# ianic/flate

Measured on AMD Instinct MI355X. Metric: MB/s uncompressed, deflate level 6 compress, higher is better.
Workload: dtype u8; 1 GPU; raw deflate level 6, 1024 MiB synthetic enwik-like text per GPU, 65535-byte independent chunks (16385 chunks), one MI355X per rank (BASELINE.json configs[1]); container=raw, chunk_bytes=65535, bytes_per_gpu=1073741824, gather=none

## Files before the change

### flate_amd/csrc/flate_hip.hip

```cpp
#include <hip/hip_runtime.h>

#include <dlfcn.h>

#include <algorithm>
#include <cstdio>
#include <cstdlib>
#include <cstring>
#include <string>
#include <chrono>
#include <deque>
#include <vector>
#include <thread>
#include <functional>

#include "../../include/flate_hip.h"
#include "kernels_block.h"
#include "kernels_common.h"
#include "kernels_deflater.h"
#include "kernels_inflate.h"
#include "kernels_inflate_par.h"
#include "kernels_inflate_size.h"
#include "kernels_lz.h"
#include "kernels_parse.h"
#include "kernels_walk.h"
// ... 15 lines not shown
    K_LZ_LINKS,
    K_LZ_WALK,
    K_LZ_EMIT,
    K_ST_PARSE,
    K_ST_EMIT,
    K_PLAN,
    K_OFFSETS,
    K_ENCODE,
    K_INFLATE,
    K_INFLATE_PAR,
    K_SPAN_SCAN,
    K_INFLATE_SPAN,
    K_INFLATE_SIZE,
    K_INFLATE_SIZE_SPAN,
    K_GATHER,
    K_INFLATER,
    K_DEFLATER,
    K_COUNT
};
const char* const kKernelNames[K_COUNT] = {"memset_out", "k_byte_hist", "k_checksum", "k_lz_sort", "k_lz_match",
                                           "k_lz_chain", "k_lz_parse", "k_lz_links", "k_lz_walk", "k_lz_emit",
                                           "k_st_parse", "k_st_emit", "k_plan",
                                           "k_offsets",  "k_encode",    "k_inflate",  "k_inflate_par", "k_span_scan", "k_inflate_span",
                                           "k_inflate_size", "k_inflate_size_span",
                                           "k_gather", "k_inflater", "k_deflater"};

struct DevBuf {
    void* p = nullptr;
    size_t cap = 0;
};

}

struct flate_hip_plan {
    std::vector<uint64_t> hin, hout;
    uint32_t n_chunks = 0;
    int container = 0, mode = 0;
    struct Pass {
        uint32_t nc = 0, nb = 0;
        void* chunks = nullptr;
        void* blk_chunk = nullptr;
    };
    std::vector<Pass> passes;
    bool ready = false;
};

struct fl_knobs {
    size_t max_pass_chunks = 32768;
    size_t host_pass_chunks = 1024;
    uint64_t stream_pass_bytes = 4096ull << 20;
    uint64_t span_min_bytes = 0;
    bool span_debug = false;
    int span_twin = -1;
    bool memset_inline = false;
    bool span_two_runs = false;
    bool no_pin_mirror = false;
    bool no_ramp = false;
    uint32_t stream_group = 0;
    int stream_windows = -1;
    bool simple_ck_inline = false;
    bool one_stream = false;
    int rect = -1;
    int64_t inflate_par = -1;
    int64_t inflate_ring = -1;
};

struct flate_hip_ctx {
    int device = 0;
    fl_knobs knobs;
    hipStream_t own_stream = nullptr;
    hipStream_t stream = nullptr;
    bool sync = true;
    uint32_t flags = 0;
    std::string last_error;
    fl_crc_consts crc{};
    DevBuf chunks, blk_chunk, plans, hist, cks, S, NC, rec, desc, marks, tokens, ntok, cflag, links, shard_sz;
    DevBuf wexit;
    DevBuf wchunks, swins;
    void* pin_in = nullptr;
    void* pin_out = nullptr;
    void* pin_len = nullptr;
    void* pin_tab = nullptr;
    size_t pin_tab_cap = 0;
    bool in_mirror = false;
    size_t pin_in_cap = 0, pin_out_cap = 0, pin_len_cap = 0;
    std::function<void(uint32_t, uint32_t)> mirror_in, mirror_out;
    uint32_t n_cu = 0;
    DevBuf sp_points, sp_found, sp_spans, sp_res, sp_cand, sp_candoff, sp_tails, sp_tails_b, sp_chain, sp_chainoff,
        sp_pool, sp_pooltab, sp_poolctl, sp_items, sp_part, sp_footoff, sp_foot, sp_fin, sp_chainpos, sp_rs;
    DevBuf tiles, segs, pieces, fpts, zones, nsorted, jmp, exitmap, entry, segtok, tokbase, bound;
    DevBuf sgroups, sgroup0, gmap, gentry, sblocks;
    DevBuf st_in, st_out, st_inoff, st_outlen, st_status, st_consumed, st_pack, st_packoff, st_slot;
    hipStream_t s_in = nullptr, s_out = nullptr;
    std::vector<hipEvent_t> xfer_events;
    hipStream_t s_ck = nullptr;
    hipEvent_t ck_ev0 = nullptr, ck_ev1 = nullptr;
    hipStream_t s_c2 = nullptr;
    hipEvent_t c2_ev0 = nullptr, c2_ev1 = nullptr;
    hipStream_t s_ms = nullptr;
    hipEvent_t ms_ev0 = nullptr, ms_ev1 = nullptr;
    bool ms_pending = false;
    bool ck_pending = false;
    uint64_t dfl_bytes = 0;
    uint64_t ws_bytes = 0;
    uint64_t dbg_span_taken = 0, dbg_span_done = 0, dbg_par_taken = 0;
    DevBuf dbg_par_handed;
    DevBuf sz_spans, sz_recs;
    uint64_t dbg_size_chain = 0, dbg_size_whole = 0;
    bool ws_fixed = false;
    uint32_t dbg_pass_chunks = 0;
    uint32_t dbg_first_chunk = 0;
    std::vector<uint64_t> dbg_pos_off;
    std::vector<fl_chunk> dbg_chunks;
    std::vector<fl_piece> dbg_pieces;
    bool prof = false;
    struct Pending {
        int kid;
        hipEvent_t a, b;
    };
    std::vector<Pending> pending;
    std::vector<hipEvent_t> free_events;
    double prof_ms[K_COUNT] = {0};
    uint64_t prof_n[K_COUNT] = {0};
};

namespace {

#define HIP_OK(h, expr)                                                                                  \
    do {                                                                                                 \
        hipError_t e_ = (expr);                                                                          \
        if (e_ != hipSuccess) {                                                                          \
            (h)->last_error = std::string(#expr) + ": " + hipGetErrorString(e_);                         \
            return FLATE_HIP_E_LAUNCH;                                                                   \
        }                                                                                                \
    } while (0)

int ensure(flate_hip_ctx* h, DevBuf& b, size_t bytes) {
    if (bytes <= b.cap) return FLATE_HIP_OK;
    if (h->ws_fixed) {
        h->last_error = "workspace of the two-stream passes too small: " + std::to_string(bytes) + " bytes asked, " +
                        std::to_string(b.cap) + " held";
        return FLATE_HIP_E_LAUNCH;
    }
    if (b.p) {
        (void)hipStreamSynchronize(h->stream);
        (void)hipFree(b.p);
        h->ws_bytes -= b.cap;
        b.p = nullptr;
        b.cap = 0;
    }
    size_t want = bytes + bytes / 8 + 256;
    hipError_t e = hipMalloc(&b.p, want);
    if (e != hipSuccess) {
        (void)hipGetLastError();
// ... 45 lines not shown
int launch_checksum_side(flate_hip_ctx* h, uint32_t nb, const uint8_t* d_in, const fl_chunk* dch, const uint32_t* dbc,
                         const fl_sblock* dsb, const fl_params& prm);

void fold_profile(flate_hip_ctx* h) {
    if (h->pending.empty()) return;
    (void)hipStreamSynchronize(h->stream);
    for (auto& p : h->pending) {
        float ms = 0;
        if (hipEventElapsedTime(&ms, p.a, p.b) == hipSuccess) {
            h->prof_ms[p.kid] += ms;
            h->prof_n[p.kid] += 1;
        }
        h->free_events.push_back(p.a);
        h->free_events.push_back(p.b);
    }
    h->pending.clear();
}

void init_crc_consts(fl_crc_consts& cc) {
    cc.xpow8[0] = 0x00800000u;
    for (int j = 1; j < 32; j++) cc.xpow8[j] = fl_crc_mulmod(cc.xpow8[j - 1], cc.xpow8[j - 1]);
    for (int m = 0; m < 64; m++) cc.pow1024[m] = fl_crc_xpow8n(cc.xpow8, 1024ull * m);
    cc.pow65535 = fl_crc_xpow8n(cc.xpow8, 65535);
}

bool level_args(int mode, fl_params& p) {
    switch (mode) {
        case 4: p.good = 4; p.lazy = 4; p.nice = 16; p.chain = 16; return true;
        case 5: p.good = 8; p.lazy = 16; p.nice = 32; p.chain = 32; return true;
        case 6: p.good = 8; p.lazy = 16; p.nice = 128; p.chain = 128; return true;
        case 7: p.good = 8; p.lazy = 32; p.nice = 128; p.chain = 256; return true;
        case 8: p.good = 32; p.lazy = 128; p.nice = 258; p.chain = 1024; return true;
        case 9: p.good = 32; p.lazy = 258; p.nice = 258; p.chain = 4096; return true;
        default: p.good = p.lazy = p.nice = p.chain = 0; return mode == 0 || mode == 1;
    }
}

void read_knobs(fl_knobs& k, uint64_t span_default) {
    k = fl_knobs();
    const char* e;
    if ((e = getenv("FLATE_HIP_MAX_PASS_CHUNKS")) && atoi(e) > 0) k.max_pass_chunks = (size_t)atoi(e);
    if ((e = getenv("FLATE_HIP_HOST_PASS_CHUNKS")) && atoi(e) > 0) k.host_pass_chunks = (size_t)atoi(e);
    if ((e = getenv("FLATE_HIP_MAX_STREAM_PASS_MIB")) && atoll(e) > 0) k.stream_pass_bytes = (uint64_t)atoll(e) << 20;
    e = getenv("FLATE_HIP_INFLATE_SPANS");
    k.span_min_bytes = e ? (uint64_t)atoll(e) : span_default;
    k.span_debug = getenv("FLATE_HIP_SPAN_DEBUG") != nullptr;
    if ((e = getenv("FLATE_HIP_SPAN_TWIN"))) k.span_twin = atoi(e);
    k.no_pin_mirror = getenv("FLATE_HIP_NO_PIN_MIRROR") != nullptr;
    k.no_ramp = getenv("FLATE_HIP_NO_RAMP") != nullptr;
    if ((e = getenv("FLATE_HIP_RECT"))) k.rect = atoi(e) != 0;
    k.one_stream = getenv("FLATE_HIP_ONE_COMPUTE_STREAM") != nullptr;
    k.simple_ck_inline = getenv("FLATE_HIP_SIMPLE_CK_INLINE") != nullptr;
    if ((e = getenv("FLATE_HIP_SPAN_TWO_RUNS"))) k.span_two_runs = atoi(e) != 0;
    if ((e = getenv("FLATE_HIP_MEMSET_INLINE"))) k.memset_inline = atoi(e) != 0;
    if ((e = getenv("FLATE_HIP_STREAM_WINDOWS"))) k.stream_windows = atoi(e) != 0;
    if ((e = getenv("FLATE_HIP_STREAM_GROUP")) && atoi(e) > 0) k.stream_group = (uint32_t)atoi(e);
    if ((e = getenv("FLATE_HIP_INFLATE_PAR"))) k.inflate_par = atoll(e);
    if ((e = getenv("FLATE_HIP_INFLATE_RING"))) k.inflate_ring = atoll(e);
}
size_t pass_chunk_limit(const flate_hip_ctx* h) { return h->knobs.max_pass_chunks; }
size_t host_pass_chunk_limit(const flate_hip_ctx* h) { return h->knobs.host_pass_chunks; }
bool is_pinned_host(const void* p) {
    hipPointerAttribute_t a;
    if (hipPointerGetAttributes(&a, p) != hipSuccess) {
        (void)hipGetLastError();
        return false;
    }
    return a.type == hipMemoryTypeHost;
}
hipError_t create_copy_stream(hipStream_t* s, bool input) {
    int least = 0, greatest = 0;
    if (hipDeviceGetStreamPriorityRange(&least, &greatest) != hipSuccess || least == greatest) {
        (void)hipGetLastError();
        return hipStreamCreateWithFlags(s, hipStreamNonBlocking);
    }
    return hipStreamCreateWithPriority(s, hipStreamNonBlocking, input ? greatest : least);
}

int xfer_event(flate_hip_ctx* h, size_t k, hipEvent_t* ev) {
    while (h->xfer_events.size() <= k) {
        hipEvent_t e;
        if (hipEventCreateWithFlags(&e, hipEventDisableTiming) != hipSuccess) return FLATE_HIP_E_ALLOC;
        h->xfer_events.push_back(e);
    }
    *ev = h->xfer_events[k];
    return FLATE_HIP_OK;
}

uint64_t stream_pass_byte_limit(const flate_hip_ctx* h) { return h->knobs.stream_pass_bytes; }

#ifndef FL_STREAM_FIX_MAX
#define FL_STREAM_FIX_MAX 3u
#endif
int compress_stream_pass(flate_hip_ctx* h, const uint8_t* d_in, const fl_params& prm, uint32_t nc, uint32_t nb,
                         const StreamTables& t, const fl_chunk* hch ) {
    hipStream_t st = h->stream;
    int rc;
    const uint32_t nseg = (uint32_t)t.segs.size(), npc = (uint32_t)t.pieces.size();
    const uint64_t npos = t.npos;
    const size_t tile_limit = pass_chunk_limit(h);
    const size_t tiles_per_launch = std::min(t.tiles.size(), tile_limit);
    if ((rc = ensure(h, h->tiles, sizeof(fl_tile) * t.tiles.size()))) return rc;
    if ((rc = ensure(h, h->segs, sizeof(fl_seg) * (t.segs.size() + 1)))) return rc;
    if ((rc = ensure(h, h->pieces, sizeof(fl_piece) * npc))) return rc;
    if ((rc = ensure(h, h->fpts, sizeof(uint32_t) * (t.fpts.size() + 1)))) return rc;
    if ((rc = ensure(h, h->zones, sizeof(uint32_t) * (t.zones.size() + 1)))) return rc;
    if ((rc = ensure(h, h->nsorted, sizeof(uint32_t) * tiles_per_launch))) return rc;
// ... 336 lines not shown
int launch_checksum_side(flate_hip_ctx* h, uint32_t nb, const uint8_t* d_in, const fl_chunk* dch, const uint32_t* dbc,
                         const fl_sblock* dsb, const fl_params& prm) {
    hipStream_t st = h->stream;
    if (!h->s_ck) {
        hipStream_t s = nullptr;
        hipEvent_t e0 = nullptr, e1 = nullptr;
        if (hipStreamCreateWithFlags(&s, hipStreamNonBlocking) != hipSuccess ||
            hipEventCreateWithFlags(&e0, hipEventDisableTiming) != hipSuccess ||
            hipEventCreateWithFlags(&e1, hipEventDisableTiming) != hipSuccess) {
            if (e0) (void)hipEventDestroy(e0);
            if (e1) (void)hipEventDestroy(e1);
            if (s) (void)hipStreamDestroy(s);
            (void)hipGetLastError();
            return FLATE_HIP_E_ALLOC;
        }
        h->s_ck = s;
        h->ck_ev0 = e0;
        h->ck_ev1 = e1;
    }
    HIP_OK(h, hipEventRecord(h->ck_ev0, st));
    HIP_OK(h, hipStreamWaitEvent(h->s_ck, h->ck_ev0, 0));
    {
        ProfScope ps(h, K_CHECKSUM, h->s_ck);
        hipLaunchKernelGGL(k_checksum, dim3(nb), dim3(64), 0, h->s_ck, d_in, dch, dbc, dsb, prm, h->crc, (uint32_t*)h->cks.p);
    }
    HIP_OK(h, hipEventRecord(h->ck_ev1, h->s_ck));
    h->ck_pending = true;
    return FLATE_HIP_OK;
}

#ifndef FL_ENC_WAVE_MIN_SLOTS_STREAM
#define FL_ENC_WAVE_MIN_SLOTS_STREAM 32768u
#endif
int enqueue_back_end(flate_hip_ctx* h, const fl_params& prm, uint32_t nc, uint32_t nb, uint32_t c0, const fl_chunk* dch,
                     const uint32_t* dbc, const fl_sblock* dsb, const uint8_t* d_in, uint8_t* d_out, uint64_t* d_outlen,
                     int32_t* d_status) {
    hipStream_t st = h->stream;
    const int mode = prm.mode;
    fl_block_plan* dpl = (fl_block_plan*)h->plans.p;
    uint32_t* dhist = (uint32_t*)h->hist.p;
    uint32_t* dcks = (uint32_t*)h->cks.p;
    {
        ProfScope ps(h, K_PLAN);
        if (mode == 0)
            hipLaunchKernelGGL(k_plan_store, dim3((nb + 255) / 256), dim3(256), 0, st, dch, dbc, dsb, nb, dpl);
        else
            hipLaunchKernelGGL(k_plan, dim3((nb + FL_PLAN_WAVES - 1) / FL_PLAN_WAVES), dim3(64 * FL_PLAN_WAVES), 0, st,
                               dch, dbc, dsb, prm, (const uint32_t*)dhist, dpl);
    }
    if (h->ck_pending) {
        HIP_OK(h, hipStreamWaitEvent(st, h->ck_ev1, 0));
        h->ck_pending = false;
    }
    if (h->ms_pending) {
        HIP_OK(h, hipStreamWaitEvent(st, h->ms_ev1, 0));
        h->ms_pending = false;
    }
    {
        ProfScope ps(h, K_OFFSETS);
        hipLaunchKernelGGL(k_offsets, dim3(nc), dim3((uint64_t)nb >= 32ull * nc ? 64 * FL_OFFS_MAX_WAVES : 64), 0, st, dch, prm, h->crc, dpl, (const uint32_t*)dcks,
                           d_out, d_outlen + c0, d_status + c0);
    }
    {
        ProfScope ps(h, K_ENCODE);
        if (mode >= 4 && nb >= (prm.stream ? FL_ENC_WAVE_MIN_SLOTS_STREAM : 8192u))
            hipLaunchKernelGGL(k_encode_wave, dim3((nb + FL_ENC_WAVES - 1) / FL_ENC_WAVES), dim3(64 * FL_ENC_WAVES), 0, st,
                               d_in, dch, dbc, (const fl_block_plan*)dpl, (const uint32_t*)h->tokens.p, (uint32_t*)d_out, nb,
                               (prm.stream || (nb & 1u)) ? 0u : 1u);
        else if (mode >= 4)
            hipLaunchKernelGGL(k_encode<true>, dim3(nb), dim3(64 * FL_ENC_WAVES), 0, st, d_in, dch, dbc,
                               (const fl_block_plan*)dpl, (const uint32_t*)h->tokens.p, (uint32_t*)d_out);
        else
            hipLaunchKernelGGL(k_encode<false>, dim3(nb), dim3(64 * FL_ENC_WAVES), 0, st, d_in, dch, dbc,
                               (const fl_block_plan*)dpl, (const uint32_t*)nullptr, (uint32_t*)d_out);
    }
    HIP_OK(h, hipGetLastError());
    return FLATE_HIP_OK;
}

int enqueue_pass(flate_hip_ctx* h, const fl_params& prm, uint32_t nc, uint32_t nb, uint32_t c0, const fl_chunk* dch,
                 const uint32_t* dbc, const fl_sblock* dsb, const uint8_t* d_in, uint8_t* d_out, uint64_t* d_outlen,
                 int32_t* d_status) {
    hipStream_t st = h->stream;
    const int mode = prm.mode, container = prm.container;
    int rc;
    fl_block_plan* dpl = (fl_block_plan*)h->plans.p;
    uint32_t* dhist = (uint32_t*)h->hist.p;
    if (container != 0 && ((mode >= 4 && prm.chain >= FL_BULK_MIN_CHAIN) || (mode < 4 && h->knobs.simple_ck_inline))) {
        ProfScope ps(h, K_CHECKSUM);
        hipLaunchKernelGGL(k_checksum, dim3(nb), dim3(64), 0, st, d_in, dch, dbc, dsb, prm, h->crc, (uint32_t*)h->cks.p);
    }
    if (container != 0 && mode < 4 && !h->knobs.simple_ck_inline && (rc = launch_checksum_side(h, nb, d_in, dch, dbc, dsb, prm))) return rc;
    if (mode >= 4) {
        if ((rc = ensure_lz_workspace(h, nc, prm.chain))) return rc;
        if (prm.chain >= FL_BULK_MIN_CHAIN) {
            HIP_OK(h, hipMemsetAsync(h->marks.p, 0, fl_lz_chunk_sizes(true).marks * nc, st));
            {
                ProfScope ps(h, K_LZ_LINKS);
                hipLaunchKernelGGL(k_lz_links<0>, dim3(nc), dim3(64 * FL_CHAIN_WAVES), 0, st, d_in, dch, (uint16_t*)h->links.p,
                                   (uint32_t*)h->cflag.p);
                hipLaunchKernelGGL(k_lz_links<1>, dim3(nc), dim3(64 * FL_CHAIN_WAVES), 0, st, d_in, dch, (uint16_t*)h->links.p,
                                   (uint32_t*)h->cflag.p);
                hipLaunchKernelGGL(k_lz_links<2>, dim3(nc), dim3(64 * FL_CHAIN_WAVES), 0, st, d_in, dch, (uint16_t*)h->links.p,
                                   (uint32_t*)h->cflag.p);
                hipLaunchKernelGGL(k_lz_links<3>, dim3(nc), dim3(64 * FL_CHAIN_WAVES), 0, st, d_in, dch, (uint16_t*)h->links.p,
                                   (uint32_t*)h->cflag.p);
            }
            {
                ProfScope ps(h, K_LZ_WALK);
                hipLaunchKernelGGL(k_lz_walk<false>, dim3(nc), dim3(WK_THREADS), 0, st, d_in, dch, prm, (const uint16_t*)h->links.p,
// ... 554 lines not shown
}

int flate_hip_create(int device, flate_hip_handle* out) {
    if (!out) return FLATE_HIP_E_INVALID_ARG;
    *out = nullptr;
    int ndev = 0;
    if (hipGetDeviceCount(&ndev) != hipSuccess || ndev <= 0 || device < 0 || device >= ndev)
        return FLATE_HIP_E_NO_DEVICE;
    if (hipSetDevice(device) != hipSuccess) return FLATE_HIP_E_NO_DEVICE;
    flate_hip_ctx* h = new flate_hip_ctx();
    h->device = device;
    if (hipStreamCreateWithFlags(&h->own_stream, hipStreamNonBlocking) != hipSuccess) {
        delete h;
        return FLATE_HIP_E_NO_DEVICE;
    }
    h->stream = h->own_stream;
    init_crc_consts(h->crc);
    read_knobs(h->knobs, FL_SPAN_MIN_BYTES);
    *out = h;
    return FLATE_HIP_OK;
}

int flate_hip_debug_reload_env(flate_hip_handle h) {
    if (!h) return FLATE_HIP_E_INVALID_ARG;
    read_knobs(h->knobs, FL_SPAN_MIN_BYTES);
    return FLATE_HIP_OK;
}

int flate_hip_destroy(flate_hip_handle h) {
    if (!h) return FLATE_HIP_E_INVALID_ARG;
    (void)hipSetDevice(h->device);
    (void)hipStreamSynchronize(h->stream);
    fold_profile(h);
    if (h->pin_in) (void)hipHostFree(h->pin_in);
    if (h->pin_len) (void)hipHostFree(h->pin_len);
    if (h->pin_tab) (void)hipHostFree(h->pin_tab);
    if (h->pin_out) (void)hipHostFree(h->pin_out);
    for (DevBuf* b : {&h->sp_points, &h->sp_found, &h->sp_spans, &h->sp_res, &h->sp_cand, &h->sp_candoff, &h->sp_tails,
                      &h->sp_tails_b, &h->sp_chain, &h->sp_chainoff, &h->sp_pool, &h->sp_pooltab, &h->sp_poolctl, &h->sp_items,
                      &h->sp_part, &h->sp_footoff, &h->sp_foot, &h->sp_fin, &h->sp_chainpos, &h->sp_rs, &h->sz_spans, &h->sz_recs})
        if (b->p) (void)hipFree(b->p);
    for (DevBuf* b : {&h->chunks, &h->blk_chunk, &h->plans, &h->hist, &h->cks, &h->S, &h->NC, &h->rec, &h->desc, &h->marks,
                      &h->tokens, &h->ntok, &h->cflag, &h->links, &h->wchunks, &h->swins, &h->wexit, &h->shard_sz, &h->tiles, &h->segs, &h->pieces, &h->fpts, &h->zones, &h->nsorted, &h->jmp,
                      &h->exitmap, &h->entry, &h->segtok, &h->tokbase, &h->bound, &h->sgroups, &h->sgroup0, &h->gmap, &h->gentry,
                      &h->sblocks, &h->st_in, &h->st_out, &h->st_inoff, &h->st_outlen, &h->st_status,
                      &h->st_consumed, &h->st_pack, &h->st_packoff, &h->st_slot, &h->dbg_par_handed})
        if (b->p) (void)hipFree(b->p);
    h->ws_bytes = 0;
    for (hipEvent_t e : h->free_events) (void)hipEventDestroy(e);
    for (hipEvent_t e : h->xfer_events) (void)hipEventDestroy(e);
    if (h->c2_ev0) (void)hipEventDestroy(h->c2_ev0);
    if (h->c2_ev1) (void)hipEventDestroy(h->c2_ev1);
    if (h->s_c2) (void)hipStreamDestroy(h->s_c2);
    if (h->ms_ev0) (void)hipEventDestroy(h->ms_ev0);
    if (h->ms_ev1) (void)hipEventDestroy(h->ms_ev1);
    if (h->s_ms) (void)hipStreamDestroy(h->s_ms);
    if (h->ck_ev0) (void)hipEventDestroy(h->ck_ev0);
    if (h->ck_ev1) (void)hipEventDestroy(h->ck_ev1);
    if (h->s_ck) (void)hipStreamDestroy(h->s_ck);
    if (h->s_in) (void)hipStreamDestroy(h->s_in);
    if (h->s_out) (void)hipStreamDestroy(h->s_out);
    (void)hipStreamDestroy(h->own_stream);
    delete h;
    return FLATE_HIP_OK;
}

int flate_hip_set_stream(flate_hip_handle h, void* hip_stream) {
    if (!h) return FLATE_HIP_E_INVALID_ARG;
    hipStream_t next = hip_stream ? (hipStream_t)hip_stream : h->own_stream;
    if (next != h->stream) {
        (void)hipSetDevice(h->device);
        (void)hipStreamSynchronize(h->stream);
        fold_profile(h);
    }
    h->stream = next;
    return FLATE_HIP_OK;
}
int flate_hip_set_sync(flate_hip_handle h, int s) {
    if (!h) return FLATE_HIP_E_INVALID_ARG;
    h->sync = s != 0;
    return FLATE_HIP_OK;
}
const char* flate_hip_last_error(flate_hip_handle h) { return h ? h->last_error.c_str() : "null handle"; }

size_t flate_hip_compress_bound(size_t n, int container, int mode) {
    (void)mode;
    const size_t hdr = container == 1 ? 18 : (container == 2 ? 6 : 0);
    return n + (n / 32768 + 2) * 16 + hdr + 64 + n / 64;
}

int flate_hip_profile_enable(flate_hip_handle h, int enable) {
    if (!h) return FLATE_HIP_E_INVALID_ARG;
    h->prof = enable != 0;
    return FLATE_HIP_OK;
}
int flate_hip_profile_reset(flate_hip_handle h) {
    if (!h) return FLATE_HIP_E_INVALID_ARG;
    fold_profile(h);
    for (int i = 0; i < K_COUNT; i++) {
        h->prof_ms[i] = 0;
        h->prof_n[i] = 0;
    }
    return FLATE_HIP_OK;
}
int flate_hip_profile_read(flate_hip_handle h, const char** names, double* total_ms, uint64_t* launches, int cap) {
    if (!h) return FLATE_HIP_E_INVALID_ARG;
    fold_profile(h);
    int n = 0;
    for (int i = 0; i < K_COUNT && n < cap; i++) {
// ... 105 lines not shown
            }
            return FLATE_HIP_OK;
        }
    }

    const uint8_t* d_in = in;
    uint8_t* d_out = out;
    uint64_t* d_outlen = out_len;
    int32_t* d_status = status;
    uint64_t in_shift = 0, out_shift = 0;
    bool pin_in = false, pin_out = false;
    if (memkind == FLATE_HIP_MEM_HOST) {
        if ((rc = ensure(h, h->st_in, (in_hi - in_lo) + 16))) return rc;
        if ((rc = ensure(h, h->st_out, (out_hi - out_lo) + 16))) return rc;
        if ((rc = ensure(h, h->st_outlen, sizeof(uint64_t) * n_chunks))) return rc;
        if ((rc = ensure(h, h->st_status, sizeof(int32_t) * n_chunks))) return rc;
        pin_in = !fs && is_pinned_host(in + in_lo);
        pin_out = !fs && is_pinned_host(out + out_lo);
        if ((pin_in && !h->s_in && create_copy_stream(&h->s_in, true) != hipSuccess) ||
            (pin_out && !h->s_out && create_copy_stream(&h->s_out, false) != hipSuccess))
            return FLATE_HIP_E_ALLOC;
        if (in_hi > in_lo && !pin_in)
            HIP_OK(h, hipMemcpyAsync(h->st_in.p, in + in_lo, in_hi - in_lo, hipMemcpyHostToDevice, st));
        d_in = (const uint8_t*)h->st_in.p;
        d_out = (uint8_t*)h->st_out.p;
        d_outlen = (uint64_t*)h->st_outlen.p;
        d_status = (int32_t*)h->st_status.p;
        in_shift = in_lo;
        out_shift = out_lo;
    } else if (((uintptr_t)out & 3) != 0) {
        return FLATE_HIP_E_INVALID_ARG;
    }

    std::vector<fl_chunk> chunks(n_chunks);
    for (uint32_t i = 0; i < n_chunks; i++) {
        fl_chunk& c = chunks[i];
        const uint64_t len = hin[i + 1] - hin[i];
        c.in_off = hin[i] - in_shift;
        c.out_off = hout[i] - out_shift;
        c.out_cap = hout[i + 1] - hout[i];
        c.skip = 0;
        if (len > (mode >= 4 ? 0xfff00000ull : 0xfffffff0ull)) return FLATE_HIP_E_INVALID_ARG;
        c.in_len = (uint32_t)len;
        c.pos_off = 0;
        c.piece0 = c.n_piece = c.flush_off = c.n_flush = c.zone_off = c.n_slides = 0;
        c.unfinished = (fs && !fs->finish) ? 1u : 0u;
        c.pad_ = 0;
    }
    if (!planning) {
        HIP_OK(h, hipMemsetAsync(d_outlen, 0, sizeof(uint64_t) * n_chunks, st));
        HIP_OK(h, hipMemsetAsync(d_status, 0, sizeof(int32_t) * n_chunks, st));
    }

    struct MsGuard {
        flate_hip_ctx* h;
        ~MsGuard() {
            if (h->ms_pending) {
                (void)hipStreamWaitEvent(h->stream, h->ms_ev1, 0);
                h->ms_pending = false;
            }
        }
    } ms_guard{h};
    if (out_hi > out_lo && !planning) {
        if (!h->s_ms) {
            hipStream_t s = nullptr;
            hipEvent_t e0 = nullptr, e1 = nullptr;
            if (hipStreamCreateWithFlags(&s, hipStreamNonBlocking) == hipSuccess && hipEventCreateWithFlags(&e0, hipEventDisableTiming) == hipSuccess &&
                hipEventCreateWithFlags(&e1, hipEventDisableTiming) == hipSuccess) {
                h->s_ms = s;
                h->ms_ev0 = e0;
                h->ms_ev1 = e1;
            } else {
                if (e0) (void)hipEventDestroy(e0);
                if (e1) (void)hipEventDestroy(e1);
                if (s) (void)hipStreamDestroy(s);
                (void)hipGetLastError();
            }
        }
        if (h->s_ms && !h->knobs.memset_inline) {
            HIP_OK(h, hipEventRecord(h->ms_ev0, st));
            HIP_OK(h, hipStreamWaitEvent(h->s_ms, h->ms_ev0, 0));
            {
                ProfScope ps(h, K_MEMSET, h->s_ms);
                HIP_OK(h, hipMemsetAsync(d_out + (out_lo - out_shift), 0, out_hi - out_lo, h->s_ms));
            }
            HIP_OK(h, hipEventRecord(h->ms_ev1, h->s_ms));
            h->ms_pending = true;
        } else {
            ProfScope ps(h, K_MEMSET);
            HIP_OK(h, hipMemsetAsync(d_out + (out_lo - out_shift), 0, out_hi - out_lo, st));
        }
    }

    fl_pass_cfg pcfg;
    pcfg.n_chunks = n_chunks;
    pcfg.host_pass_chunks = host_pass_chunk_limit(h);
    pcfg.max_pass_chunks = pass_chunk_limit(h);
    pcfg.pinned = pin_in || pin_out;
    pcfg.ramp = !h->knobs.no_ramp;
    pcfg.planned = pl != nullptr;
    const size_t pass_limit = fl_pass_limit(pcfg);
    const uint64_t stream_pass_bytes = stream_pass_byte_limit(h);
    if (pin_out) HIP_OK(h, hipStreamSynchronize(h->s_out));
    uint8_t* zc_out = nullptr;
    std::vector<uint64_t> zc_slot;
    if (pin_out && out_hi > out_lo) {
        void* dp = nullptr;
        if (hipHostGetDevicePointer(&dp, out + out_lo, 0) == hipSuccess && dp) {
            zc_out = (uint8_t*)dp;
            zc_slot.resize((size_t)n_chunks + 1);
            for (uint32_t i = 0; i <= n_chunks; i++) zc_slot[i] = hout[i] - out_lo;
            if ((rc = ensure(h, h->st_slot, sizeof(uint64_t) * ((size_t)n_chunks + 1)))) return rc;
            HIP_OK(h, hipMemcpyAsync(h->st_slot.p, zc_slot.data(), sizeof(uint64_t) * ((size_t)n_chunks + 1), hipMemcpyHostToDevice, st));
        } else {
            (void)hipGetLastError();
        }
    }
    const bool pinned_passes = (pin_in || pin_out) && !pl;
    uint64_t blk_total = 0, blk_base = 0;
    if (pinned_passes) {
        if (!h->s_in && create_copy_stream(&h->s_in, true) != hipSuccess) return FLATE_HIP_E_ALLOC;
        for (uint32_t i = 0; i < n_chunks; i++)
            blk_total += mode >= 4 ? 2u : (uint64_t)(chunks[i].in_len / FL_BLOCK_BYTES + 1);
        if ((rc = ensure(h, h->chunks, sizeof(fl_chunk) * (size_t)n_chunks))) return rc;
        if ((rc = ensure(h, h->blk_chunk, sizeof(uint32_t) * (size_t)std::max<uint64_t>(blk_total, 1)))) return rc;
        HIP_OK(h, hipStreamSynchronize(h->s_in));
        const size_t tab_need = sizeof(fl_chunk) * (size_t)n_chunks + sizeof(uint32_t) * (size_t)std::max<uint64_t>(blk_total, 1);
        if (h->pin_tab_cap < tab_need) {
            if (h->pin_tab) (void)hipHostFree(h->pin_tab);
            h->pin_tab = nullptr;
            h->pin_tab_cap = 0;
            const size_t sz = tab_need + tab_need / 4 + 4096;
            if (hipHostMalloc(&h->pin_tab, sz, hipHostMallocDefault) != hipSuccess) {
                (void)hipGetLastError();
                h->pin_tab = nullptr;
                return FLATE_HIP_E_ALLOC;
            }
            h->pin_tab_cap = sz;
        }
    }
    uint32_t nc = 0;
    size_t pass_count = 0;
    std::deque<std::vector<uint32_t>> keep_blk;
    std::deque<std::vector<fl_sblock>> keep_sb;
    struct PassGuard {
        flate_hip_ctx* h;
        bool on;
        ~PassGuard() {
            if (on) {
                if (h->s_in) (void)hipStreamSynchronize(h->s_in);
                if (h->s_c2) (void)hipStreamSynchronize(h->s_c2);
                (void)hipStreamSynchronize(h->stream);
            }
            h->ck_pending = false;
        }
    } pass_guard{h, pinned_passes};
    const bool planned_run = pl && pl->ready;
    bool two = ((pinned_passes && (size_t)n_chunks > pass_limit) || (planned_run && pl->passes.size() > 1)) && mode >= 4 && !fs && !h->knobs.one_stream;
    for (uint32_t i = 0; two && i < n_chunks; i++) two = chunks[i].in_len <= FLATE_HIP_MAX_LZ_CHUNK;
    if (two && !h->s_c2) {
        hipStream_t s2 = nullptr;
        hipEvent_t e0 = nullptr, e1 = nullptr;
        if (hipStreamCreateWithFlags(&s2, hipStreamNonBlocking) == hipSuccess && hipEventCreateWithFlags(&e0, hipEventDisableTiming) == hipSuccess &&
            hipEventCreateWithFlags(&e1, hipEventDisableTiming) == hipSuccess) {
            h->s_c2 = s2;
            h->c2_ev0 = e0;
            h->c2_ev1 = e1;
        } else {
            if (e0) (void)hipEventDestroy(e0);
            if (e1) (void)hipEventDestroy(e1);
            if (s2) (void)hipStreamDestroy(s2);
            (void)hipGetLastError();
            two = false;
        }
    }
    std::vector<fl_pass> sched;
    uint64_t slice_nc = 0, slice_nb = 0;
    auto size_two_slices = [&](uint64_t nc_, uint64_t nb_) -> int {
        int r;
        if ((r = ensure_lz_workspace(h, (uint32_t)(2 * nc_), prm.chain))) return r;
        return ensure_block_workspace(h, 2 * nb_);
    };
    if (two) {
        if (planned_run) {
            for (size_t k = 0; k < pl->passes.size(); k++) {
                fl_pass p;
                p.c0 = sched.empty() ? 0 : sched.back().c0 + sched.back().nc;
                p.nc = pl->passes[k].nc;
                p.stream = (uint32_t)(k & 1u);
                sched.push_back(p);
                slice_nc = std::max<uint64_t>(slice_nc, pl->passes[k].nc);
                slice_nb = std::max<uint64_t>(slice_nb, pl->passes[k].nb);
            }
        } else {
            slice_nc = fl_pass_schedule(pcfg, sched);
            slice_nb = 2 * slice_nc;
            if (sched.size() < 2) two = false;
        }
        if (two && size_two_slices(slice_nc, slice_nb)) {
            (void)hipGetLastError();
            two = false;
        }
    }
    pass_guard.on = pinned_passes || two;
    struct WsFixed {
        flate_hip_ctx* h;
        ~WsFixed() { h->ws_fixed = false; }
    } ws_fixed{h};
    h->ws_fixed = two;
    if (two) {
        HIP_OK(h, hipEventRecord(h->c2_ev0, st));
        HIP_OK(h, hipStreamWaitEvent(h->s_c2, h->c2_ev0, 0));
        if (h->ms_pending) HIP_OK(h, hipStreamWaitEvent(h->s_c2, h->ms_ev1, 0));
    }
    struct WsShift {
        std::vector<std::pair<DevBuf*, size_t>> undo;
        void add(DevBuf& b, size_t bytes) {
            b.p = (uint8_t*)b.p + bytes;
            b.cap -= bytes;
            undo.emplace_back(&b, bytes);
        }
        ~WsShift() {
            for (auto& u : undo) {
                u.first->p = (uint8_t*)u.first->p - u.second;
                u.first->cap += u.second;
            }
        }
    };
    auto enqueue_sliced = [&](size_t k, uint32_t nc_, uint32_t nb_, uint32_t c0_, const fl_chunk* dch_, const uint32_t* dbc_,
                              const fl_sblock* dsb_) -> int {
        if (k >= sched.size() || sched[k].c0 != c0_ || sched[k].nc != nc_ || nc_ > slice_nc || nb_ > slice_nb) {
            h->last_error = "two-stream pass " + std::to_string(k) + " (" + std::to_string(c0_) + " + " + std::to_string(nc_) +
                            " chunks) is not the scheduled one";
            return FLATE_HIP_E_LAUNCH;
        }
        const uint32_t slice = sched[k].stream;
        hipStream_t sq = slice ? h->s_c2 : st;
        WsShift ws;
        const size_t c_sl = (size_t)slice * slice_nc, b0 = (size_t)slice * slice_nb;
        const bool bulk = prm.chain >= FL_BULK_MIN_CHAIN;
        const fl_lz_sizes z = fl_lz_chunk_sizes(bulk);
        const fl_blk_sizes bs = fl_block_slot_sizes();
        ws.add(h->plans, bs.plan * b0);
        ws.add(h->hist, bs.hist * b0);
        ws.add(h->cks, bs.cks * b0);
        ws.add(bulk ? h->links : h->S, z.links * c_sl);
        ws.add(h->desc, z.desc * c_sl);
        ws.add(h->marks, z.marks * c_sl);
        ws.add(h->tokens, z.tokens * c_sl);
        ws.add(h->ntok, z.ntok * c_sl);
        ws.add(h->cflag, z.cflag * c_sl);
        hipStream_t saved = h->stream;
        h->stream = sq;
        const int r = enqueue_pass(h, prm, nc_, nb_, c0_, dch_, dbc_, dsb_, d_in, d_out, d_outlen, d_status);
        h->stream = saved;
        return r;
    };
    std::vector<uint32_t> pass_c0;
    const bool landing = pin_out && (bool)h->mirror_out;
    if (landing && h->pin_len_cap < sizeof(uint64_t) * (size_t)n_chunks) {
        if (h->pin_len) (void)hipHostFree(h->pin_len);
        h->pin_len = nullptr;
        h->pin_len_cap = 0;
        const size_t sz = sizeof(uint64_t) * ((size_t)n_chunks + n_chunks / 4 + 64);
        if (hipHostMalloc(&h->pin_len, sz, hipHostMallocDefault) != hipSuccess) {
            (void)hipGetLastError();
// ... 1480 lines not shown
```

### flate_amd/csrc/kernels_block.h

```cpp
#pragma once
#include "kernels_common.h"

struct fl_sb {
    uint32_t start, len;
    bool final_block, marker;
};
__device__ __forceinline__ fl_sb fl_simple_block(const fl_chunk& ck, const fl_sblock* __restrict__ sblocks, uint32_t b) {
    fl_sb r;
    if (sblocks) {
        const fl_sblock e = sblocks[b];
        r.start = e.start;
        r.len = e.len;
        r.final_block = (e.flags & 1) != 0;
        r.marker = (e.flags & 2) != 0;
    } else {
        const uint32_t j = b - ck.first_block;
        const uint64_t s = (uint64_t)j * FL_BLOCK_BYTES;
        r.start = (uint32_t)min(s, (uint64_t)ck.in_len);
        r.len = min(FL_BLOCK_BYTES, ck.in_len - r.start);
        r.final_block = j + 1 == ck.n_blocks;
        r.marker = false;
    }
    return r;
}
// ... 373 lines not shown
                        m.has = 1;
                    } else {
                        m.a = plan->size_bits;
                    }
                }
            }
            fl_offmap inc = m;
#pragma unroll
            for (int d = 1; d < 64; d <<= 1) {
                fl_offmap o;
                o.a = __shfl_up(inc.a, d, 64);
                o.c = __shfl_up(inc.c, d, 64);
                o.has = __shfl_up(inc.has, d, 64);
                if (lane >= (uint32_t)d) inc = fl_offmap_compose(o, inc);
            }
            if (write) {
                fl_offmap exc;
                exc.a = __shfl_up(inc.a, 1, 64);
                exc.c = __shfl_up(inc.c, 1, 64);
                exc.has = __shfl_up(inc.has, 1, 64);
                if (lane == 0) exc = ident;
                if (plan && plan->valid) {
                    plan->bit_off = fl_offmap_apply(fl_offmap_compose(run, exc), base);
                    if (plan->q1_gap && j + 1 < ck.n_blocks) {
                        const fl_block_plan* nx = &plans[ck.first_block + j + 1];
                        if (nx->valid && (plan->type == FL_BLOCK_STORED) != (nx->type == FL_BLOCK_STORED)) q1_sh = 1u;
                    }
                }
            }
            fl_offmap last;
            last.a = __shfl(inc.a, 63, 64);
            last.c = __shfl(inc.c, 63, 64);
            last.has = __shfl(inc.has, 63, 64);
            run = fl_offmap_compose(run, last);
        }
        return run;
    };
    fl_offmap run;
    if (W == 1) {
        run = pass(ident, true);
    } else {
        const fl_offmap mine = pass(ident, false);
        if (lane == 0) wtot[wave] = mine;
        __syncthreads();
        fl_offmap pre = ident;
        for (uint32_t x = 0; x < wave; x++) pre = fl_offmap_compose(pre, wtot[x]);
        run = pass(pre, true);
        for (uint32_t x = wave + 1; x < W; x++) run = fl_offmap_compose(run, wtot[x]);
    }
    const uint64_t end_bits = fl_offmap_apply(run, base);
    const uint64_t body_end = (end_bits + 7) >> 3;
    const uint64_t total = body_end + ftr_bytes - ck.out_off;
    const bool fits = total <= ck.out_cap;

    uint32_t cks = 0;
    if (prm.container != 0 && threadIdx.x == 0) {
        if (prm.mode >= 4 && !prm.stream) {
            cks = cks_part[2 * (uint64_t)ck.first_block];
            if (prm.container == 2) {
                const uint32_t A = cks & 0xffff, B = cks >> 16, n = ck.in_len;
                const uint32_t a = (1 + A) % 65521u;
                const uint32_t bsum = (uint32_t)(((uint64_t)n + B) % 65521u);
                cks = a | (bsum << 16);
            }
        }
    }
    if (prm.container != 0 && !(prm.mode >= 4 && !prm.stream)) {
        const uint32_t nbw = r1 - r0, per = (nbw + 63) / 64;
        const uint32_t j0 = r0 + min(lane * per, nbw), j1 = min(j0 + per, r1);
        uint32_t x = 0, y = 0, len = 0;
        for (uint32_t j = j0; j < j1; j++) {
            const uint32_t pc = cks_part[2 * (uint64_t)(ck.first_block + j)];
            const uint32_t pl = cks_part[2 * (uint64_t)(ck.first_block + j) + 1];
            if (prm.container == 1) {
                const uint32_t shf = pl == FL_BLOCK_BYTES ? cc.pow65535 : fl_crc_xpow8n(cc.xpow8, pl);
                x = fl_crc_mulmod(x, shf) ^ pc;
            } else {
                y = (uint32_t)(((uint64_t)y + (uint64_t)x * pl + (pc >> 16)) % 65521u);
                x = (x + (pc & 0xffff)) % 65521u;
            }
            len += pl;
        }
        const uint32_t incl = fl_wave_incl_scan_dpp(len);
        if (lane == 63) wl[wave] = incl;
        __syncthreads();
        uint32_t before = 0, all = 0;
        for (uint32_t w = 0; w < W; w++) {
            if (w < wave) before += (uint32_t)wl[w];
            all += (uint32_t)wl[w];
        }
        const uint32_t behind = all - (before + incl);
        uint32_t px, py = 0;
        if (prm.container == 1) {
            px = fl_wave_xor(len ? fl_crc_mulmod(x, fl_crc_xpow8n(cc.xpow8, behind)) : 0u);
        } else {
            px = fl_wave_sum(x);
            py = fl_wave_sum((uint32_t)(((uint64_t)y + (uint64_t)x * (behind % 65521u)) % 65521u));
        }
        if (lane == 0) {
            wx[wave] = px;
            wy[wave] = py;
        }
        __syncthreads();
        if (threadIdx.x == 0) {
            uint32_t fx = 0, fy = 0;
            for (uint32_t w = 0; w < W; w++) {
// ... 113 lines not shown
                                                              uint32_t* __restrict__ out32) {
    __shared__ uint32_t lit_lds[FL_NUM_LIT + 2];
    __shared__ uint32_t dist_lds[FL_NUM_DIST + 2];
    __shared__ uint32_t wave_bits[FL_ENC_WAVES];
    __shared__ uint32_t stg[FL_ENC_WAVES][FL_STG_DW];

    const uint32_t b = blockIdx.x;
    const fl_block_plan* plan = &plans[b];
    if (!plan->valid) return;
    const uint32_t cidx = blk_chunk[b];
    const fl_chunk ck = chunks[cidx];
    const uint32_t tid = threadIdx.x, lane = tid & 63, wave = tid >> 6;
    const uint64_t bit_off = plan->bit_off;
    const uint8_t* src = in + ck.in_off;

    if (plan->type == FL_BLOCK_STORED) {
        const uint32_t len = plan->in_len;
        const uint64_t p = (bit_off + 3 + 7) >> 3;
        if (tid == 0) {
            if (plan->final_block) fl_atomic_or_bits(out32, bit_off, 1, 1);
            const uint32_t lw = (len & 0xffff) | ((~len & 0xffff) << 16);
            fl_atomic_or_bits(out32, p * 8, lw, 32);
        }
        fl_copy_bytes(out32, p + 4, src + plan->in_start, len, tid, 64 * FL_ENC_WAVES);
        return;
    }

    for (uint32_t i = tid; i < FL_NUM_LIT; i += 64 * FL_ENC_WAVES)
        lit_lds[i] = (uint32_t)plan->lit[i].code | ((uint32_t)plan->lit[i].len << 16);
    if (tid < FL_NUM_DIST) dist_lds[tid] = (uint32_t)plan->dist[tid].code | ((uint32_t)plan->dist[tid].len << 16);
    for (uint32_t i = lane; i < FL_STG_DW; i += 64) stg[wave][i] = 0;
    __syncthreads();

    const uint32_t hdr_nbits = plan->hdr_nbits;
    const uint32_t n_hdr = (hdr_nbits + 7) >> 3;
    const uint32_t n_sym = plan->tok_count;
    const uint32_t n_items = n_hdr + FL_ENC_UNITS(TOKENS, n_sym) + 1;
    const uint8_t* bytes = src + plan->tok_start;
    const uint32_t* toks = TOKENS ? tokens + ck.pos_off + plan->tok_start : nullptr;
    const uint8_t* hdr = plan->hdr;

    uint32_t per = (n_items + FL_ENC_WAVES - 1) / FL_ENC_WAVES;
    per = (per + 63) & ~63u;
    const uint32_t i0 = min(n_items, wave * per), i1 = min(n_items, i0 + per);

    uint32_t nb = 0;
    for (uint32_t i = i0 + lane; i < i1; i += 64)
        nb += fl_block_item<TOKENS>(i, n_hdr, hdr_nbits, n_sym, hdr, bytes, toks, lit_lds, dist_lds).n;
    nb = fl_wave_sum(nb);
    if (lane == 0) wave_bits[wave] = nb;
    __syncthreads();
    uint64_t cur = bit_off;
    for (uint32_t w = 0; w < wave; w++) cur += wave_bits[w];
    if (i0 >= i1) return;

    const uint64_t first_dw = cur >> 5;
    uint32_t* sw = stg[wave];
    for (uint32_t ib = i0; ib < i1; ib += 64) {
        const uint32_t i = ib + lane;
        fl_item it;
        it.v = 0;
        it.n = 0;
        if (i < i1) it = fl_block_item<TOKENS>(i, n_hdr, hdr_nbits, n_sym, hdr, bytes, toks, lit_lds, dist_lds);
        const uint32_t incl = fl_wave_incl_scan(it.n, lane);
        const uint32_t total = __shfl(incl, 63, 64);
        const uint64_t base_dw = cur >> 5;
        if (it.n) {
            const uint32_t rel = (uint32_t)(cur - (base_dw << 5)) + (incl - it.n);
            const uint32_t dw = rel >> 5, sh = rel & 31;
            const uint64_t a = it.v << sh;
            const uint32_t hi = sh ? (uint32_t)(it.v >> (64 - sh)) : 0u;
            if ((uint32_t)a) atomicOr(&sw[dw], (uint32_t)a);
            if ((uint32_t)(a >> 32)) atomicOr(&sw[dw + 1], (uint32_t)(a >> 32));
            if (hi) atomicOr(&sw[dw + 2], hi);
        }
        fl_lds_order();
        const uint64_t end = cur + total;
        const uint32_t nd = (uint32_t)((end >> 5) - base_dw);
        for (uint32_t k = lane; k < nd; k += 64) {
            const uint32_t v = sw[k];
            if (base_dw + k == first_dw) {
                if (v) atomicOr(&out32[base_dw + k], v);
            } else {
                out32[base_dw + k] = v;
            }
        }
        const uint32_t carry = sw[nd];
        fl_lds_order();
        for (uint32_t k = lane; k <= nd + 2 && k < FL_STG_DW; k += 64) sw[k] = 0;
        fl_lds_order();
        if (lane == 0) sw[0] = carry;
        fl_lds_order();
        cur = end;
    }
    if ((cur & 31) && lane == 0) {
        const uint32_t v = sw[0];
        if (v) atomicOr(&out32[cur >> 5], v);
    }
}

__global__ __launch_bounds__(64 * FL_ENC_WAVES) void k_encode_wave(const uint8_t* __restrict__ in,
                                                              const fl_chunk* __restrict__ chunks,
                                                              const uint32_t* __restrict__ blk_chunk,
                                                              const fl_block_plan* __restrict__ plans,
                                                              const uint32_t* __restrict__ tokens ,
                                                              uint32_t* __restrict__ out32, uint32_t n_blocks,
// ... 230 lines not shown
```

### flate_amd/engine.py

```python
import ctypes as C
import os

import numpy as np

from . import _capi
from ._capi import FlateHipError, MEM_DEVICE, MEM_HOST


class Engine:
    def __init__(self, device=0):
        self._L = _capi.lib()
        self._h = C.c_void_p()
        rc = self._L.flate_hip_create(int(device), C.byref(self._h))
        if rc != 0:
            import sys
            hint = ""
            if "torch" in sys.modules and os.environ.get("FLATE_HIP_PRELOAD_TORCH_HIP", "0") in ("", "0"):
                hint = ("; this process also runs PyTorch, which ships its own libamdhip64: import torch BEFORE flate_amd, "
                        "or set FLATE_HIP_PRELOAD_TORCH_HIP=1 before importing flate_amd, so that both use one runtime")
            raise FlateHipError("flate_hip_create(device=%d) failed with %d: no usable MI355X / HIP device "
                                "(there is no CPU fallback)%s" % (device, rc, hint))
        self.device = device

    def close(self):
        if getattr(self, "_h", None) and self._h.value:
            self._L.flate_hip_destroy(self._h)
            self._h = C.c_void_p()

    def __del__(self):
        try:
            self.close()
        except Exception:
            pass

    def _check(self, rc, what):
        if rc != 0:
            err = self._L.flate_hip_last_error(self._h).decode()
            raise FlateHipError("%s failed with %d (%s)" % (what, rc, err))

    _KNOBS = ("FLATE_HIP_MAX_PASS_CHUNKS", "FLATE_HIP_HOST_PASS_CHUNKS", "FLATE_HIP_MAX_STREAM_PASS_MIB",
              "FLATE_HIP_INFLATE_SPANS", "FLATE_HIP_SPAN_DEBUG", "FLATE_HIP_SPAN_TWIN", "FLATE_HIP_NO_PIN_MIRROR",
              "FLATE_HIP_NO_RAMP", "FLATE_HIP_INFLATE_PAR", "FLATE_HIP_INFLATE_RING", "FLATE_HIP_RECT", "FLATE_HIP_STREAM_WINDOWS", "FLATE_HIP_SIMPLE_CK_INLINE", "FLATE_HIP_STREAM_GROUP", "FLATE_HIP_SPAN_TWO_RUNS", "FLATE_HIP_MEMSET_INLINE", "FLATE_HIP_ONE_COMPUTE_STREAM")

    def _sync_env(self):
        now = tuple(os.environ.get(k) for k in self._KNOBS)
        if now != getattr(self, "_knob_state", None):
            if getattr(self, "_knob_state", None) is not None or any(v is not None for v in now):
                self._L.flate_hip_debug_reload_env(self._h)
            self._knob_state = now

    def set_stream(self, stream_ptr):
        self._L.flate_hip_set_stream(self._h, C.c_void_p(stream_ptr or 0))

    def set_sync(self, flag):
        self._L.flate_hip_set_sync(self._h, int(bool(flag)))

    def set_flags(self, flags):
        self._check(self._L.flate_hip_set_flags(self._h, int(flags)), "flate_hip_set_flags")

    def compress_bound(self, n, container=0, mode=6):
        return self._L.flate_hip_compress_bound(int(n), container, mode)

    def compress_many(self, chunks, container=0, mode=6):
        self._sync_env()
        n = len(chunks)
        if n == 0:
            return [], []
        lens = np.array([len(c) for c in chunks], dtype=np.uint64)
        in_off = np.zeros(n + 1, dtype=np.uint64)
        np.cumsum(lens, out=in_off[1:])
        blob = np.frombuffer(b"".join(bytes(c) for c in chunks), dtype=np.uint8)
        if blob.size == 0:
            blob = np.zeros(1, dtype=np.uint8)
        caps = np.array([(self.compress_bound(int(l), container, mode) + 7) & ~7 for l in lens], dtype=np.uint64)
        out_off = np.zeros(n + 1, dtype=np.uint64)
        np.cumsum(caps, out=out_off[1:])
        out = np.zeros(int(out_off[-1]) + 8, dtype=np.uint8)
        out_len = np.zeros(n, dtype=np.uint64)
        status = np.zeros(n, dtype=np.int32)
        rc = self._L.flate_hip_compress_batch(self._h, blob.ctypes.data, in_off.ctypes.data, n, container, mode,
                                              out.ctypes.data, out_off.ctypes.data, out_len.ctypes.data,
                                              status.ctypes.data, MEM_HOST)
        self._check(rc, "flate_hip_compress_batch")
        res = [out[int(out_off[i]): int(out_off[i]) + int(out_len[i])].tobytes() for i in range(n)]
        return res, [int(s) for s in status]

    def compress_flush(self, data, flush_points, finish=True, container=0, mode=6):
        self._sync_env()
        blob = np.frombuffer(bytes(data), dtype=np.uint8) if len(data) else np.zeros(1, dtype=np.uint8)
        fp = np.array(list(flush_points), dtype=np.uint64)
        cap = (self.compress_bound(len(data), container, mode) + 64 * (len(fp) + 1) + 7) & ~7
        out = np.zeros(cap + 8, dtype=np.uint8)
        out_len = np.zeros(1, dtype=np.uint64)
        status = np.zeros(1, dtype=np.int32)
        rc = self._L.flate_hip_compress_flush(self._h, blob.ctypes.data, len(data), fp.ctypes.data if len(fp) else None,
# ... 368 lines not shown
```

Before: 42780 MB/s.

## Replace whole-output memset with targeted zeroing of boundary dwords in kernels

Removes the side-stream memset of the entire device output range and instead has the offsets kernel and encode kernels zero only the dwords that are OR-written at block and wave boundaries. The intent is to avoid writing the full output buffer (about a GiB) twice and to drop the cross-stream event waits. A host-memory path keeps a memset. The risk is that any dword that is OR-accumulated but not covered by the new zeroing produces corrupt output, and the extra __syncthreads adds a little kernel overhead.

```diff
diff --git a/flate_amd/csrc/flate_hip.hip b/flate_amd/csrc/flate_hip.hip
--- a/flate_amd/csrc/flate_hip.hip
+++ b/flate_amd/csrc/flate_hip.hip
@@ -91,7 +91,6 @@
     uint64_t span_min_bytes = 0;
     bool span_debug = false;
     int span_twin = -1;
-    bool memset_inline = false;
     bool span_two_runs = false;
     bool no_pin_mirror = false;
     bool no_ramp = false;
@@ -136,9 +135,6 @@
     hipEvent_t ck_ev0 = nullptr, ck_ev1 = nullptr;
     hipStream_t s_c2 = nullptr;
     hipEvent_t c2_ev0 = nullptr, c2_ev1 = nullptr;
-    hipStream_t s_ms = nullptr;
-    hipEvent_t ms_ev0 = nullptr, ms_ev1 = nullptr;
-    bool ms_pending = false;
     bool ck_pending = false;
     uint64_t dfl_bytes = 0;
     uint64_t ws_bytes = 0;
@@ -290,7 +286,6 @@
     k.one_stream = getenv("FLATE_HIP_ONE_COMPUTE_STREAM") != nullptr;
     k.simple_ck_inline = getenv("FLATE_HIP_SIMPLE_CK_INLINE") != nullptr;
     if ((e = getenv("FLATE_HIP_SPAN_TWO_RUNS"))) k.span_two_runs = atoi(e) != 0;
-    if ((e = getenv("FLATE_HIP_MEMSET_INLINE"))) k.memset_inline = atoi(e) != 0;
     if ((e = getenv("FLATE_HIP_STREAM_WINDOWS"))) k.stream_windows = atoi(e) != 0;
     if ((e = getenv("FLATE_HIP_STREAM_GROUP")) && atoi(e) > 0) k.stream_group = (uint32_t)atoi(e);
     if ((e = getenv("FLATE_HIP_INFLATE_PAR"))) k.inflate_par = atoll(e);
@@ -733,10 +728,6 @@
         HIP_OK(h, hipStreamWaitEvent(st, h->ck_ev1, 0));
         h->ck_pending = false;
     }
-    if (h->ms_pending) {
-        HIP_OK(h, hipStreamWaitEvent(st, h->ms_ev1, 0));
-        h->ms_pending = false;
-    }
     {
         ProfScope ps(h, K_OFFSETS);
         hipLaunchKernelGGL(k_offsets, dim3(nc), dim3((uint64_t)nb >= 32ull * nc ? 64 * FL_OFFS_MAX_WAVES : 64), 0, st, dch, prm, h->crc, dpl, (const uint32_t*)dcks,
@@ -1397,9 +1388,6 @@
     if (h->c2_ev0) (void)hipEventDestroy(h->c2_ev0);
     if (h->c2_ev1) (void)hipEventDestroy(h->c2_ev1);
     if (h->s_c2) (void)hipStreamDestroy(h->s_c2);
-    if (h->ms_ev0) (void)hipEventDestroy(h->ms_ev0);
-    if (h->ms_ev1) (void)hipEventDestroy(h->ms_ev1);
-    if (h->s_ms) (void)hipStreamDestroy(h->s_ms);
     if (h->ck_ev0) (void)hipEventDestroy(h->ck_ev0);
     if (h->ck_ev1) (void)hipEventDestroy(h->ck_ev1);
     if (h->s_ck) (void)hipStreamDestroy(h->s_ck);
@@ -1611,46 +1599,6 @@
         HIP_OK(h, hipMemsetAsync(d_status, 0, sizeof(int32_t) * n_chunks, st));
     }
 
-    struct MsGuard {
-        flate_hip_ctx* h;
-        ~MsGuard() {
-            if (h->ms_pending) {
-                (void)hipStreamWaitEvent(h->stream, h->ms_ev1, 0);
-                h->ms_pending = false;
-            }
-        }
-    } ms_guard{h};
-    if (out_hi > out_lo && !planning) {
-        if (!h->s_ms) {
-            hipStream_t s = nullptr;
-            hipEvent_t e0 = nullptr, e1 = nullptr;
-            if (hipStreamCreateWithFlags(&s, hipStreamNonBlocking) == hipSuccess && hipEventCreateWithFlags(&e0, hipEventDisableTiming) == hipSuccess &&
-                hipEventCreateWithFlags(&e1, hipEventDisableTiming) == hipSuccess) {
-                h->s_ms = s;
-                h->ms_ev0 = e0;
-                h->ms_ev1 = e1;
-            } else {
-                if (e0) (void)hipEventDestroy(e0);
-                if (e1) (void)hipEventDestroy(e1);
-                if (s) (void)hipStreamDestroy(s);
-                (void)hipGetLastError();
-            }
-        }
-        if (h->s_ms && !h->knobs.memset_inline) {
-            HIP_OK(h, hipEventRecord(h->ms_ev0, st));
-            HIP_OK(h, hipStreamWaitEvent(h->s_ms, h->ms_ev0, 0));
-            {
-                ProfScope ps(h, K_MEMSET, h->s_ms);
-                HIP_OK(h, hipMemsetAsync(d_out + (out_lo - out_shift), 0, out_hi - out_lo, h->s_ms));
-            }
-            HIP_OK(h, hipEventRecord(h->ms_ev1, h->s_ms));
-            h->ms_pending = true;
-        } else {
-            ProfScope ps(h, K_MEMSET);
-            HIP_OK(h, hipMemsetAsync(d_out + (out_lo - out_shift), 0, out_hi - out_lo, st));
-        }
-    }
-
     fl_pass_cfg pcfg;
     pcfg.n_chunks = n_chunks;
     pcfg.host_pass_chunks = host_pass_chunk_limit(h);
@@ -1675,6 +1623,10 @@
             (void)hipGetLastError();
         }
     }
+    if (memkind == FLATE_HIP_MEM_HOST && out_hi > out_lo && !planning && !(zc_out && h->knobs.rect != 1)) {
+        ProfScope ps(h, K_MEMSET);
+        HIP_OK(h, hipMemsetAsync(d_out, 0, out_hi - out_lo, st));
+    }
     const bool pinned_passes = (pin_in || pin_out) && !pl;
     uint64_t blk_total = 0, blk_base = 0;
     if (pinned_passes) {
@@ -1770,7 +1722,6 @@
     if (two) {
         HIP_OK(h, hipEventRecord(h->c2_ev0, st));
         HIP_OK(h, hipStreamWaitEvent(h->s_c2, h->c2_ev0, 0));
-        if (h->ms_pending) HIP_OK(h, hipStreamWaitEvent(h->s_c2, h->ms_ev1, 0));
     }
     struct WsShift {
         std::vector<std::pair<DevBuf*, size_t>> undo;
diff --git a/flate_amd/csrc/kernels_block.h b/flate_amd/csrc/kernels_block.h
--- a/flate_amd/csrc/kernels_block.h
+++ b/flate_amd/csrc/kernels_block.h
@@ -449,6 +449,33 @@
     const uint64_t body_end = (end_bits + 7) >> 3;
     const uint64_t total = body_end + ftr_bytes - ck.out_off;
     const bool fits = total <= ck.out_cap;
+
+    __syncthreads();
+    if (fits) {
+        const uint64_t lo = ck.out_off, hi = ck.out_off + ck.out_cap;
+        auto zero_dw = [&](uint64_t dw) {
+            const uint64_t b = dw << 2;
+            if (b >= lo && b + 4 <= hi) {
+                *(uint32_t*)(out + b) = 0u;
+            } else {
+                for (uint32_t k = 0; k < 4; k++)
+                    if (b + k >= lo && b + k < hi) out[b + k] = 0;
+            }
+        };
+        for (uint32_t j = threadIdx.x; j < ck.n_blocks; j += blockDim.x) {
+            const fl_block_plan* plan = &plans[ck.first_block + j];
+            if (!plan->valid) continue;
+            const uint64_t bo = plan->bit_off;
+            if (plan->type == FL_BLOCK_STORED) {
+                const uint64_t p = (bo + 3 + 7) >> 3;
+                for (uint64_t dw = bo >> 5; dw <= (p + 4) >> 2; dw++) zero_dw(dw);
+                if (plan->in_len) zero_dw((p + 4 + plan->in_len - 1) >> 2);
+            } else {
+                zero_dw(bo >> 5);
+                zero_dw((bo + plan->size_bits - 1) >> 5);
+            }
+        }
+    }
 
     uint32_t cks = 0;
     if (prm.container != 0 && threadIdx.x == 0) {
@@ -668,6 +695,11 @@
     __syncthreads();
     uint64_t cur = bit_off;
     for (uint32_t w = 0; w < wave; w++) cur += wave_bits[w];
+    {
+        const uint64_t blk_first = bit_off >> 5, blk_last = (bit_off + plan->size_bits - 1) >> 5;
+        if (wave && i0 < i1 && lane == 0 && (cur >> 5) != blk_first && (cur >> 5) != blk_last) out32[cur >> 5] = 0u;
+    }
+    __syncthreads();
     if (i0 >= i1) return;
 
     const uint64_t first_dw = cur >> 5;
diff --git a/flate_amd/engine.py b/flate_amd/engine.py
--- a/flate_amd/engine.py
+++ b/flate_amd/engine.py
@@ -40,7 +40,7 @@
 
     _KNOBS = ("FLATE_HIP_MAX_PASS_CHUNKS", "FLATE_HIP_HOST_PASS_CHUNKS", "FLATE_HIP_MAX_STREAM_PASS_MIB",
               "FLATE_HIP_INFLATE_SPANS", "FLATE_HIP_SPAN_DEBUG", "FLATE_HIP_SPAN_TWIN", "FLATE_HIP_NO_PIN_MIRROR",
-              "FLATE_HIP_NO_RAMP", "FLATE_HIP_INFLATE_PAR", "FLATE_HIP_INFLATE_RING", "FLATE_HIP_RECT", "FLATE_HIP_STREAM_WINDOWS", "FLATE_HIP_SIMPLE_CK_INLINE", "FLATE_HIP_STREAM_GROUP", "FLATE_HIP_SPAN_TWO_RUNS", "FLATE_HIP_MEMSET_INLINE", "FLATE_HIP_ONE_COMPUTE_STREAM")
+              "FLATE_HIP_NO_RAMP", "FLATE_HIP_INFLATE_PAR", "FLATE_HIP_INFLATE_RING", "FLATE_HIP_RECT", "FLATE_HIP_STREAM_WINDOWS", "FLATE_HIP_SIMPLE_CK_INLINE", "FLATE_HIP_STREAM_GROUP", "FLATE_HIP_SPAN_TWO_RUNS", "FLATE_HIP_ONE_COMPUTE_STREAM")
 
     def _sync_env(self):
         now = tuple(os.environ.get(k) for k in self._KNOBS)
```

Measured after the change: 42890 MB/s, median of 6. About the same (+0.2%).
